# openai/whisper

Hardware: AMD Instinct MI355X
Metric: audio-seconds transcribed per wall-second (large-v3 greedy) (higher is better)
Workload: dtype f16

## Files before the change

### include/whisper_hip.h

```cpp
#ifndef WHISPER_HIP_H
#define WHISPER_HIP_H

#include <stddef.h>
#include <stdint.h>

#ifdef __cplusplus
extern "C" {
#endif

#define WH_ABI_VERSION 1
#define WH_MEL_SCRATCH_BYTES 2048

enum {
  WH_OK = 0,
  WH_ERR_ARG = 1,
  WH_ERR_WORKSPACE = 2,
  WH_ERR_HIP = 3,
  WH_ERR_STATE = 4,
  WH_ERR_LIMIT = 5,
  WH_ERR_HANDOFF = 6,
  WH_RUNNING = 7,
  WH_ERR_STREAM = 8
};

// ... 61 lines not shown
                          int64_t *n_frames_out, int32_t *stats, void *scratch, size_t scratch_bytes, void *stream);

int wh_model_create(const wh_dims *dims, int dtype, const wh_model_weights *weights, wh_model **out);
void wh_model_destroy(wh_model *m);

size_t wh_encoder_workspace_bytes(const wh_model *m, int batch);
int wh_encode(const wh_model *m, const void *mel, int mel_is_f16, int batch, void *out,
              void *workspace, size_t workspace_bytes, void *stream);

enum {
  WH_TASK_CAPTURE_Q = 1,
  WH_TASK_TWO_LAUNCH_SELF = 2,
  WH_TASK_TWO_LAUNCH_CROSS = 4,
  WH_TASK_EXPIRE_HANDOFFS = 16,
  WH_TASK_FUSED_SELF = 32,
  WH_TASK_LN_PROLOGUE = 64
};
size_t wh_task_workspace_bytes(const wh_model *m, int n_audio, int n_group, int max_prefill_tokens,
                               int flags);
int wh_task_create(const wh_model *m, int n_audio, int n_group, int max_prefill_tokens, int flags,
                   void *workspace, size_t workspace_bytes, wh_task **out);
void wh_task_destroy(wh_task *t);
int wh_task_set_audio(wh_task *t, const void *features, void *stream);
int wh_task_prefill(wh_task *t, const int64_t *tokens, int64_t token_stride, int T0,
                    const int32_t *sel_pos, int n_sel, float *logits_out, void *stream);
size_t wh_score_scratch_bytes(const wh_model *m, int n_rows, int n_pos);
int wh_task_score(wh_task *t, const int64_t *tokens, int64_t token_stride, int T0, const int32_t *n_tok,
                  int first, int v_end, float *logprob_out, float *top_logprob_out, int32_t *top_token_out,
                  void *scratch, size_t scratch_bytes, void *stream);
int wh_task_step(wh_task *t, const int64_t *last_tokens, int64_t token_stride, float *logits_out,
                 void *stream);
// ... 89 lines not shown
```

### whisper_amd/csrc/api.cpp

```cpp
#include "../../include/whisper_hip.h"
#include "kernels.h"
#include "flac_core.h"

#include <hip/hip_runtime.h>
#include <math.h>
#include <cmath>
#include <stdlib.h>
#include <string.h>
#include <atomic>
#include <mutex>
#include <new>
#include <vector>

using namespace whk;

static thread_local hipError_t g_last_hip = hipSuccess;

#define HIPCHK(expr)                                   \
  do {                                                 \
    hipError_t _e = (expr);                            \
    if (_e != hipSuccess) { g_last_hip = _e; return WH_ERR_HIP; } \
  } while (0)

extern "C" int wh_abi_version(void) { return WH_ABI_VERSION; }
// ... 207 lines not shown
    HIPCHK(gemm(m, w.att, D, L.out_w, D, w.x, D, M, D, L.out_b, 0, w.x, D, true, s));
    HIPCHK(launch_layernorm(w.x, D, L.mlp_ln_w, L.mlp_ln_b, w.xn, D, M, D, m->dtype, s));
    HIPCHK(gemm(m, w.xn, D, L.fc1_w, D, w.h, 4 * D, M, 4 * D, L.fc1_b, 1, nullptr, 0, false, s));
    HIPCHK(gemm(m, w.h, 4 * D, L.fc2_w, 4 * D, w.x, D, M, D, L.fc2_b, 0, w.x, D, true, s));
  }
  HIPCHK(launch_layernorm(w.x, D, m->w.enc_ln_post_w, m->w.enc_ln_post_b, out, D, M, D, m->dtype, s));
  return WH_OK;
}

struct wh_loop;
struct wh_task {
  const wh_model* m;
  int B, G, R, Tmax, flags;
  int pos;
  bool audio_set;
  int steps_eager[2];
  int handoff_fallbacks;
  hipGraph_t graph[2]; hipGraphExec_t graph_exec[2];
  void* cross_kv;
  void* cross_vt;
  int vt_ld;
  void* self_k; void* self_v;
  void* spare_k; void* spare_v;
  float* x; void* xn; void* qkv; void* att; void* h; void* qbuf;
  void* part_o; float* part_ml;
  float* logits;
  float* xsel; void* xseln;
  int* d_pos; int* d_alive; int* d_sel; int* d_src;
  int* d_lag;
  int* h_lag;
  int* h_poll;
  hipEvent_t poll_event;
  hipEvent_t done_event;
// ... 29 lines not shown
};

enum { LOOP_IDLE = 0, LOOP_GREEDY = 1, LOOP_BEAM = 2 };
enum { PH_STEPPING = 0, PH_DRAINING = 1 };
struct wh_loop {
  int phase;
  hipStream_t s;
  wh_beam_params bp;
  int64_t* tokens; int64_t token_stride; int sot_index, no_speech_token;
  float* sum_logprobs; float* no_speech_probs;
  int64_t* fin_tokens; int32_t* fin_len; float* fin_scores; int32_t* fin_count;
  SampleArgs sa; BeamArgs ba;
  PhraseArgs ph; bool biased;
  RepArgs rep; bool rep_on;
  bool fused_embed, pending, wait_due;
  int ntok, steps, ntok_at_copy, cur;
  int n_tokens;
};

struct TaskGuard {
  wh_task* t; bool ok;
  explicit TaskGuard(wh_task* task, bool loop_call = false) : t(task), ok(false) {
    if (t) {
      int expected = 0; ok = t->busy.compare_exchange_strong(expected, 1);
      if (ok && !loop_call && t->loop_kind != 0) { t->busy.store(0); ok = false; }
    }
  }
  ~TaskGuard() { if (t && ok) t->busy.store(0); }
};
#define TASK_ENTER(task) TaskGuard _guard(task); if ((task) && !_guard.ok) return WH_ERR_STATE
// ... 42 lines not shown
  t->qbuf = c.take(R * D * es);
  size_t Rp = Mx < (size_t)SKINNY_ROWS ? Mx : (size_t)SKINNY_ROWS;
  if (Rp < R) Rp = R;
  if (Rp < 48) Rp = 48;
  t->part_o = c.take(Rp * H * DEC_ATTN_MAX_SPLITS * 64 * 4);
  t->part_ml = (float*)c.take(Rp * H * DEC_ATTN_MAX_SPLITS * 2 * 4);
  t->logits = (float*)c.take(R * 2 * V * 4);
  t->xsel = (float*)c.take(Mx * D * 4);
  t->xseln = c.take(Mx * D * es);
  t->d_pos = (int*)c.take(256);
  t->d_alive = (int*)c.take(256);
  t->d_sel = (int*)c.take(Mx * 4);
  t->d_src = (int*)c.take(R * 4);
  t->d_lag = (int*)c.take(R * 4);
  t->step_tokens = (int64_t*)c.take(R * 8);
  t->samp_part = (float*)c.take(greedy_sample_scratch_bytes((int)R, (int)V));
  t->samp_state = (int*)c.take(R * 16);
  t->phrase_root = (int*)c.take(V * 4);
  t->phrase_span = (int*)c.take(R * 8);
  t->beam_scratch = t->G > 1 ? c.take(beam_scratch_bytes((int)R, (int)V)) : nullptr;
  t->beam_flags = t->G > 1 ? (int*)c.take((2 * (size_t)t->B + 1) * 4) : nullptr;
  t->beam_lcp = t->G > 1 ? (int*)c.take(((size_t)t->B * 64 + R) * 4) : nullptr;
  t->qcap = (t->flags & WH_TASK_CAPTURE_Q) ? c.take(L * R * C * D * es) : nullptr;
  t->xq_gran = (unsigned long long*)c.take(R * (D / 2) * 8);
  t->sq_gran = (unsigned long long*)c.take(R * (3 * D / 2) * 8);
  t->so_gran = (unsigned long long*)c.take(R * (D / 2) * 8);
  t->x2 = (float*)c.take(R * D * 4);
  t->d_tick = (int*)c.take(256);
  t->d_err = t->d_tick + 16;
  t->merge_cnt = (int*)c.take(R * H * 4);
  t->xh = c.take((R + 7) / 8 * 8 * D * 2);
// ... 38 lines not shown
#ifdef WH_DEV
    t->fused_out = t->fused_sattn && (WH_DEV_FLAG("WH_FUSED_OUT") || (flags & 8 ));
#else
    t->fused_out = false;
#endif
  }
  t->h_lag = (int*)calloc((size_t)t->R, sizeof(int));
  if (!t->h_lag) { delete t; return WH_ERR_ARG; }
  t->needs_reset = true;
  t->busy.store(0);
  *out = t;
  return WH_OK;
}

static void drop_step_graphs(wh_task* t) {
  for (int i = 0; i < 2; ++i) {
    if (t->graph_exec[i]) { (void)hipGraphExecDestroy(t->graph_exec[i]); t->graph_exec[i] = nullptr; }
    if (t->graph[i]) { (void)hipGraphDestroy(t->graph[i]); t->graph[i] = nullptr; }
    t->steps_eager[i] = 0;
  }
}

extern "C" void wh_task_destroy(wh_task* t) {
  if (!t) return;
  drop_step_graphs(t);
  free(t->h_lag);
  if (t->h_poll) (void)hipHostFree(t->h_poll);
  if (t->h_sel) (void)hipHostFree(t->h_sel);
  if (t->poll_event) (void)hipEventDestroy(t->poll_event);
  if (t->done_event) (void)hipEventDestroy(t->done_event);
  if (t->sel_event) (void)hipEventDestroy(t->sel_event);
  delete t->loop;
  delete t;
}

extern "C" int wh_task_position(const wh_task* t) { return t ? t->pos : -1; }

extern "C" int wh_task_info(wh_task* t, int what, void* stream) {
  if (!t) return -1;
  if (what == 0) return t->fused_xattn ? 1 : 0;
  if (what == 2) return t->fused_sattn ? 1 : 0;
  if (what == 3) return (t->fused_out || t->fused_xout) ? 1 : 0;
  if (what == 4) return t->handoff_fallbacks;
  if (what == 5) return t->ln_post_sites;
  if (what == 1) {
    if (t->needs_reset) return 0;
    int v = 0;
    if (hipMemcpyAsync(&v, t->d_err, 4, hipMemcpyDeviceToHost, (hipStream_t)stream) != hipSuccess) return -1;
    if (hipStreamSynchronize((hipStream_t)stream) != hipSuccess) return -1;
    return v;
  }
  return -1;
}

static int task_reset_impl(wh_task* t, void* stream_) {
  if (!t) return WH_ERR_ARG;
  hipStream_t s = (hipStream_t)stream_;
  HIPCHK(hipMemsetAsync(t->d_pos, 0, 4, s));
  t->pos = 0;
// ... 430 lines not shown
static SAttnArgs sattn_args(const wh_task* t, int l, int epoch, const float* x_in, float* x_out) {
  const wh_model* m = t->m;
  const wh_dims& d = m->d;
  const int D = d.n_text_state;
  const wh_layer_weights& L = m->dec[l];
  SAttnArgs a; memset(&a, 0, sizeof(a));
  a.xf = x_in; a.xf_ld = D; a.W = L.qkv_w; a.bias = L.qkv_b; a.D = D; a.H = d.n_text_head; a.R = t->R;
  a.out_w = L.out_w; a.out_b = L.out_b; a.x_out = x_out; a.og = t->so_gran;
  a.kcache = self_k_layer(t, l); a.vcache = self_v_layer(t, l); a.cache_bs = (int64_t)d.n_text_ctx * D;
  a.d_pos = t->d_pos; a.lag = t->d_lag; a.q_out = t->qbuf;
  a.out = t->att; a.o_ld = D;
  a.qg = t->sq_gran; a.d_tick = t->d_tick; a.epoch = epoch; a.layer = l; a.err = t->d_err; a.mode = fused_mode(1) | ((t->flags & WH_TASK_EXPIRE_HANDOFFS) ? 4 : 0);
  return a;
}

static int step_launch(wh_task* t, hipStream_t s, bool embedded = false) {
  const wh_model* m = t->m;
  const wh_dims& d = m->d;
  const int D = d.n_text_state, C = d.n_text_ctx, V = d.n_vocab;
  const int R = t->R;
  if (!embedded)
    HIPCHK(launch_embed(t->step_tokens, 1, R, 1, m->w.tok_emb, m->w.dec_pos, t->d_pos, t->d_lag, D, V, t->x, m->dtype, s));
  float* xc = t->x;
  float* xo = t->x2;
  const StepPlan plan = step_plan(t);
  t->ln_post_sites = (int)plan.post_cq + (int)plan.post_fc1;
  for (int l = 0; l < d.n_text_layer; ++l) {
    const wh_layer_weights& L = m->dec[l];
    bool out_done = false;
    if (t->fused_sattn) {
      HIPCHK(launch_sattn8(sattn_args(t, l, 0, xc, t->fused_out ? xo : nullptr), s));
// ... 9 lines not shown
    if (t->fused_xout) out_done = true;
    if (!out_done)
      HIPCHK(gemv_resid(m, plain_proj(t, t->att, D, plan.frag_self, t->self_splits, R, L.out_w, L.out_b, D, D), xc, s,
                        plan.post_cq ? t : nullptr));
    if (t->fused_xattn) {
      HIPCHK(launch_xattn8(xattn_args(t, l, 0, xc, t->fused_xout), s));
    } else {
      HIPCHK(gemv_store(m, ln_site(t, plan.post_cq, false, xc, L.cross_ln_w, L.cross_ln_b, L.cq_w, L.cq_b, D), EPI_STORE, t->qbuf, D, false, s));
      HIPCHK(launch_attn_decode(cross_attn_args(t, l, t->qbuf, R, t->G, t->cross_splits, &plan), m->dtype, s));
    }
    const int rc = launch_cross_out(t, plan, L, xc, s);
    if (rc != WH_OK) return rc;
    HIPCHK(gemv_store(m, ln_site(t, plan.post_fc1, false, xc, L.mlp_ln_w, L.mlp_ln_b, L.fc1_w, L.fc1_b, 4 * D), EPI_GELU, t->h, 4 * D, plan.frag_mlp, s));
    HIPCHK(gemv_resid(m, plain_proj(t, t->h, 4 * D, plan.frag_mlp, 1, R, L.fc2_w, L.fc2_b, D, 4 * D), xc, s));
  }
  GemvArgs g = logits_proj(m, xc, R, t->logits, V);
  g.bump = t->d_pos; g.bump_by = 1;
  g.bump2 = t->d_tick;
  HIPCHK(launch_gemv(g, m->dtype, s));
  return WH_OK;
}

static bool graphs_enabled() {
  static int v = -1;
  if (v < 0) { const char* e = getenv("WH_NO_GRAPH"); v = (e && e[0] == '1') ? 0 : 1; }
  return v == 1;
}

static int step_run(wh_task* t, hipStream_t s, bool embedded = false) {
  if (t->pos <= 0) return WH_ERR_STATE;
  if (t->pos + 1 > t->m->d.n_text_ctx) return WH_ERR_ARG;
  int rc;
  const int gi = embedded ? 1 : 0;
  if (t->graph_exec[gi]) {
    HIPCHK(hipGraphLaunch(t->graph_exec[gi], s));
  } else if (s == nullptr || !graphs_enabled() || t->steps_eager[gi] < 1) {
    rc = step_launch(t, s, embedded);
    if (rc != WH_OK) return rc;
    t->steps_eager[gi]++;
  } else {
    HIPCHK(hipStreamBeginCapture(s, hipStreamCaptureModeThreadLocal));
    rc = step_launch(t, s, embedded);
    hipError_t e = hipStreamEndCapture(s, &t->graph[gi]);
    if (rc != WH_OK) return rc;
    HIPCHK(e);
    HIPCHK(hipGraphInstantiate(&t->graph_exec[gi], t->graph[gi], nullptr, nullptr, 0));
    HIPCHK(hipGraphLaunch(t->graph_exec[gi], s));
  }
  t->pos += 1;
  return WH_OK;
}

extern "C" int wh_task_step(wh_task* t, const int64_t* last_tokens, int64_t token_stride, float* logits_out,
                            void* stream_) {
  TASK_ENTER(t);
  if (!t || !last_tokens || !logits_out) return WH_ERR_ARG;
  hipStream_t s = (hipStream_t)stream_;
// ... 100 lines not shown
  HIPCHK(hipMemcpyAsync(t->h_poll + t->B + HP_ERR0, t->d_err, 4, hipMemcpyDeviceToHost, s));

  int32_t sel[2]; int n_sel;
  const bool want_ns = L->no_speech_token >= 0 && L->no_speech_probs != nullptr;
  if (want_ns && L->sot_index != T0 - 1) { sel[0] = L->sot_index; sel[1] = T0 - 1; n_sel = 2; }
  else { sel[0] = T0 - 1; n_sel = 1; }
  int rc = prefill_impl(t, L->tokens, L->token_stride, T0, sel, n_sel, t->logits, V, s, leaders);
  if (rc != WH_OK) return rc;
  if (leaders) { rc = replicate_leader_rows(t, T0, t->logits, n_sel, s); if (rc != WH_OK) return rc; }
  if (want_ns) HIPCHK(launch_no_speech(t->logits, (int64_t)n_sel * V, R, V, L->no_speech_token, L->no_speech_probs, s));
  HIPCHK(hipMemsetAsync(L->sum_logprobs, 0, (size_t)R * 4, s));
  *n_sel_out = n_sel;
  return WH_OK;
}

static int greedy_start(wh_task* t) {
  wh_loop* L = t->loop;
  hipStream_t s = L->s;
  const wh_greedy_params* p = &L->bp.rules;
  const wh_dims& d = t->m->d;
  const int V = d.n_vocab, R = t->R, T0 = p->sample_begin;
  int* hp = t->h_poll + t->B;
  int n_sel;
  int rc = loop_prompt_pass(t, false, &n_sel);
  if (rc != WH_OK) return rc;
  hp[HP_ALIVE_INIT] = T0 - 1;
  HIPCHK(hipMemcpyAsync(t->d_alive, hp + HP_ALIVE_INIT, 4, hipMemcpyHostToDevice, s));

  SampleArgs& sa = L->sa; memset(&sa, 0, sizeof(sa));
  set_sampling_rules(sa.rules, t, L);
// ... 10 lines not shown
    HIPCHK(hipMemsetAsync(t->phrase_span, 0, (size_t)R * 8, s));
  }
  L->rep_on = t->rep_on; L->rep = t->rep;
  L->fused_embed = !WH_DEV_FLAG("WH_NO_FUSED_EMBED");
  if (L->fused_embed) {
    sa.x_next = t->x; sa.tok_emb = t->m->w.tok_emb; sa.pos_emb = t->m->w.dec_pos; sa.D = d.n_text_state;
    sa.emb_f16 = t->m->dtype == WH_F16 ? 1 : 0; sa.n_pos = d.n_text_ctx;
  }
  if (p->temperature > 0.f) {
    sa.inv_temperature = 1.0f / p->temperature;
    sa.seed_lo = (uint32_t)(p->seed & 0xffffffffu); sa.seed_hi = (uint32_t)(p->seed >> 32);
  }
  sa.rules.logits = t->logits + (size_t)(n_sel - 1) * V; sa.rules.logits_ld = (int64_t)n_sel * V;
  HIPCHK(launch_greedy_sample(sa, s, L->biased ? &ph : nullptr, L->rep_on ? &L->rep : nullptr));
  sa.rules.logits = t->logits; sa.rules.logits_ld = V;
  L->ntok = T0 + 1; L->steps = 1;
  L->pending = L->wait_due = false; L->ntok_at_copy = 0;
  L->phase = PH_STEPPING;
  return WH_OK;
}

static int beam_update(wh_task* t, const float* logits, int64_t logits_ld, int first) {
  wh_loop* L = t->loop;
  const wh_dims& d = t->m->d;
  const size_t es = t->m->esize;
  const int R = t->R, B = t->B, G = t->G;
  const int64_t row_bytes = (int64_t)d.n_text_ctx * d.n_text_state * es;
  int64_t* buf[2] = {L->tokens, L->tokens + (int64_t)R * L->token_stride};
  int* done[2] = {t->beam_flags, t->beam_flags + B};
  BeamArgs& a = L->ba;
// ... 54 lines not shown
      bool finished = false;
      for (;;) {
        if (L->pending && L->wait_due) {
          const int rc = event_reached(t->poll_event, block);
          if (rc != WH_OK) return rc;
          L->pending = L->wait_due = false;
          if (t->loop_kind == LOOP_GREEDY) {
            if (t->h_poll[0] < L->ntok_at_copy - 1) { finished = true; break; }
          } else {
            bool fin = true;
            for (int b = 0; b < B; ++b) fin = fin && t->h_poll[b] != 0;
            if (fin) { finished = true; break; }
          }
        }
        if (!(L->steps < p->max_steps && L->ntok <= p->n_ctx && L->ntok <= d.n_text_ctx)) break;
        int rc = step_run(t, s, t->loop_kind == LOOP_GREEDY && L->fused_embed);
        if (rc != WH_OK) return rc;
        if (t->loop_kind == LOOP_GREEDY) HIPCHK(launch_greedy_sample(L->sa, s, L->biased ? &L->ph : nullptr, L->rep_on ? &L->rep : nullptr));
        else { rc = beam_update(t, t->logits, d.n_vocab, 0); if (rc != WH_OK) return rc; }
        ++L->ntok; ++L->steps;
        if (L->pending && (L->steps & 7) == 2) L->wait_due = true;
        if ((L->steps & 7) == 0) {
          if (t->loop_kind == LOOP_GREEDY) HIPCHK(hipMemcpyAsync(t->h_poll, t->d_alive, 4, hipMemcpyDeviceToHost, s));
          else HIPCHK(hipMemcpyAsync(t->h_poll, (L->cur ? t->beam_flags + B : t->beam_flags), (size_t)B * 4, hipMemcpyDeviceToHost, s));
          HIPCHK(hipEventRecord(t->poll_event, s));
          L->pending = true; L->wait_due = false; L->ntok_at_copy = L->ntok;
        }
      }
      (void)finished;
      if (t->loop_kind == LOOP_GREEDY) {
        HIPCHK(hipMemcpyAsync(hp + HP_ALIVE, t->d_alive, 4, hipMemcpyDeviceToHost, s));
      } else {
        HIPCHK(hipMemcpyAsync(hp + HP_APPLIED, t->beam_flags + 2 * B, 4, hipMemcpyDeviceToHost, s));
// ... 529 lines not shown
```

### whisper_amd/csrc/gemv.hip

```cpp
#include "common.h"
#include "kernels.h"
#include <stdlib.h>

#ifndef WH_GEMV8_MAX_ROWS
#define WH_GEMV8_MAX_ROWS 24
#endif

namespace {

#define ISSUE_FENCE() asm volatile("" ::: "memory")

constexpr int CS = 4;

__device__ __forceinline__ float4v load_part4(const float* p) { return *(const float4v*)p; }
__device__ __forceinline__ float4v load_part4(const half_t* p) {
  const half4v h = *(const half4v*)p;
  return float4v{(float)h[0], (float)h[1], (float)h[2], (float)h[3]};
}

template <typename T> struct Pack4;
template <> struct Pack4<float> {
  static __device__ __forceinline__ void store(float* p, float a, float b, float c, float d) {
    *(float4v*)p = float4v{a, b, c, d};
  }
// ... 1191 lines not shown
bool rows48_applies(const whk::GemvArgs& a) {
  return !WH_DEV_FLAG("WH_NO_ROWS48") && a.R > WH_GEMV8_MAX_ROWS && a.R <= 48 && a.pro == whk::PRO_LN && a.ln_folded &&
         a.K % 256 == 0 && a.K <= 1280 && a.N >= 2048 && a.variant <= 0 &&
         (a.epi == whk::EPI_STORE || a.epi == whk::EPI_GELU || a.epi == whk::EPI_QKV);
}

hipError_t launch_rows48(const whk::GemvArgs& a, hipStream_t stream) {
  whk::g_form = "rows48";
  const size_t lds = (size_t)48 * a.K * 2 > 49152 ? (size_t)48 * a.K * 2 : 49152;
  static whk::LdsAttr attr2;
  { hipError_t e = whk::raise_dynamic_lds(attr2, (const void*)gemv_rows48_kernel<2>, 160 * 1024); if (e != hipSuccess) return e; }
  hipLaunchKernelGGL((gemv_rows48_kernel<2>), dim3((a.N + 31) / 32), dim3(1024), lds, stream, a);
  return hipGetLastError();
}

__global__ __launch_bounds__(1024) void gemv_rows48_stream_kernel(whk::GemvArgs a) {
  extern __shared__ __attribute__((aligned(16))) char smem[];
  pin_kernargs(a);
  constexpr int WAVES = 16, J = 5, NB = 20;
  const int K = a.K, nks = K / 32;
  half_t* xs = (half_t*)smem;
  float* gb = (float*)(smem + (size_t)48 * K * 2);
  const int tid = threadIdx.x, lane = tid & 63;
  const int wave = __builtin_amdgcn_readfirstlane(tid >> 6);
  const int i16 = lane & 15, g4 = lane >> 4;
  const int R = a.R;
  const int ntiles = (a.N + 15) / 16;

  float4v v[3][J];
#pragma unroll
  for (int i = 0; i < 3; ++i) {
    const int r = wave + WAVES * i;
    const float* src = a.xf + (int64_t)(r < R ? r : 0) * a.xf_ld;
#pragma unroll
    for (int j = 0; j < J; ++j) {
      int k = (j * 64 + lane) * 4; if (k > K - 4) k = K - 4;
      v[i][j] = *(const float4v*)(src + k);
    }
  }
  for (int k = tid * 4; k < K; k += 4096) {
    *(float4v*)(gb + k) = *(const float4v*)(a.ln_w + k);
    *(float4v*)(gb + K + k) = *(const float4v*)(a.ln_b + k);
  }
  __syncthreads();
  {
    const float invK = 1.0f / (float)K;
#pragma unroll
    for (int i = 0; i < 3; ++i) {
      const int r = wave + WAVES * i;
      float sum = 0.f;
#pragma unroll
      for (int j = 0; j < J; ++j) {
        const float t = (v[i][j][0] + v[i][j][1]) + (v[i][j][2] + v[i][j][3]);
        sum += ((j * 64 + lane) * 4 < K) ? t : 0.f;
      }
      const float mean = wave_sum(sum) * invK;
      float ss = 0.f;
// ... 11 lines not shown
        const int k = (j * 64 + lane) * 4;
        if (k < K) {
          const float4v w4 = *(const float4v*)(gb + k), b4 = *(const float4v*)(gb + K + k);
          half_t* dst = xr + ((((k >> 3) ^ (r & 15)) << 3) | (k & 7));
          if (r < R)
            Pack4<half_t>::store(dst, (v[i][j][0] - mean) * rstd * w4[0] + b4[0], (v[i][j][1] - mean) * rstd * w4[1] + b4[1],
                                 (v[i][j][2] - mean) * rstd * w4[2] + b4[2], (v[i][j][3] - mean) * rstd * w4[3] + b4[3]);
          else
            Pack4<half_t>::store(dst, 0.f, 0.f, 0.f, 0.f);
        }
      }
    }
  }
  __syncthreads();

  for (int tile = blockIdx.x * WAVES + wave; tile < ntiles; tile += gridDim.x * WAVES) {
    int n = tile * 16 + i16; if (n > a.N - 1) n = a.N - 1;
    const half_t* base = (const half_t*)a.W + (int64_t)n * K + g4 * 8;
    float4v acc[3];
#pragma unroll
    for (int rt = 0; rt < 3; ++rt) acc[rt] = float4v{0.f, 0.f, 0.f, 0.f};
    for (int st0 = 0; st0 < nks; st0 += NB) {
      half8v w[NB];
#pragma unroll
      for (int u = 0; u < NB; ++u) {
        int st = st0 + u; if (st > nks - 1) st = nks - 1;
        w[u] = __builtin_nontemporal_load((const half8v*)(base + st * 32));
      }
#pragma unroll
      for (int u = 0; u < NB; ++u) {
        const int st = st0 + u;
        if (st < nks) {
#pragma unroll
          for (int rt = 0; rt < 3; ++rt) {
            const half8v xf = *(const half8v*)(xs + (size_t)(rt * 16 + i16) * K + (((st * 4 + g4) ^ i16) << 3));
            acc[rt] = __builtin_amdgcn_mfma_f32_16x16x32_f16(w[u], xf, acc[rt], 0, 0, 0);
          }
        }
      }
    }
#pragma unroll
    for (int rt = 0; rt < 3; ++rt) {
      const int row = rt * 16 + i16;
      if (row < R) {
        float* y = (float*)a.y + (int64_t)row * a.y_ld + tile * 16 + g4 * 4;
#pragma unroll
        for (int e = 0; e < 4; ++e)
          if (tile * 16 + g4 * 4 + e < a.N) y[e] = acc[rt][e];
      }
    }
  }
  if (a.bump && blockIdx.x == 0 && tid == 0) atomicAdd(a.bump, a.bump_by);
  if (a.bump2 && blockIdx.x == 0 && tid == 0) atomicAdd(a.bump2, 1);
}

bool rows48_stream_applies(const whk::GemvArgs& a) {
  return !WH_DEV_FLAG("WH_NO_ROWS48") && a.R > 16 && a.R <= 48 && a.pro == whk::PRO_LN && a.epi == whk::EPI_F32 && !a.bias &&
         a.K % 256 == 0 && a.K <= 1280 && a.N >= 16384 && a.variant <= 0;
}

hipError_t launch_rows48_stream(const whk::GemvArgs& a, hipStream_t stream) {
  whk::g_form = "rows48_stream";
  const size_t lds = (size_t)48 * a.K * 2 + (size_t)2 * a.K * 4;
  static whk::LdsAttr attr;
  { hipError_t e = whk::raise_dynamic_lds(attr, (const void*)gemv_rows48_stream_kernel, 160 * 1024); if (e != hipSuccess) return e; }
  const int ntiles = (a.N + 15) / 16;
  int wgs = (ntiles + 15) / 16;
  if (wgs > 256) wgs = 256;
  hipLaunchKernelGGL(gemv_rows48_stream_kernel, dim3(wgs), dim3(1024), lds, stream, a);
  return hipGetLastError();
}

template <typename T, int MS>
__global__ __launch_bounds__(256) void merge_partials_kernel(const T* __restrict__ part_o, const float* __restrict__ part_ml,
                                                             int S, int R, int H, T* __restrict__ out, int64_t o_ld, int o_frag) {
  const int i = blockIdx.x * 256 + threadIdx.x;
  if (i >= R * H * 16) return;
  const int r = i / (H * 16), rem = i - r * (H * 16);
  const int h = rem >> 4, d4 = rem & 15;
  const int64_t pb = (int64_t)r * H + h, ps = (int64_t)R * H;
  float2v ml[MS];
  float4v o[MS];
#pragma unroll
  for (int s = 0; s < MS; ++s) {
// ... 87 lines not shown
  g_form = dtype == 1 ? (splits <= 4 ? "merge<half,4>" : "merge<half,16>") : (splits <= 4 ? "merge<float,4>" : "merge<float,16>");
  if (dtype == 1) {
    if (splits <= 4)
      hipLaunchKernelGGL((merge_partials_kernel<half_t, 4>), grid, block, 0, stream, (const half_t*)part_o, part_ml, splits, R, H, (half_t*)out, o_ld, o_frag);
    else
      hipLaunchKernelGGL((merge_partials_kernel<half_t, DEC_ATTN_MAX_SPLITS>), grid, block, 0, stream, (const half_t*)part_o, part_ml, splits, R, H, (half_t*)out, o_ld, o_frag);
  } else {
    if (splits <= 4)
      hipLaunchKernelGGL((merge_partials_kernel<float, 4>), grid, block, 0, stream, (const float*)part_o, part_ml, splits, R, H, (float*)out, o_ld, o_frag);
    else
      hipLaunchKernelGGL((merge_partials_kernel<float, DEC_ATTN_MAX_SPLITS>), grid, block, 0, stream, (const float*)part_o, part_ml, splits, R, H, (float*)out, o_ld, o_frag);
  }
  return hipGetLastError();
}

}
```

### whisper_amd/csrc/kernels.h

```cpp
#pragma once
#include <hip/hip_runtime.h>
#include <stdint.h>

#ifdef WH_PROBE
#define WH_PROBE_FIELD long long* probe;
#define WH_PROBE_KVHS_FIELD int64_t kv_hs;
#define WH_PROBE_AT(args, wg, i) \
  do { if ((args).probe && threadIdx.x == 0) (args).probe[(size_t)(wg) * 8 + (i)] = clock64(); } while (0)
#else
#define WH_PROBE_FIELD
#define WH_PROBE_KVHS_FIELD
#define WH_PROBE_AT(args, wg, i) do {} while (0)
#endif

#ifdef WH_DEV
#include <stdlib.h>
#define WH_DEV_FLAG(name) ([] { static const bool v = [] { const char* e = getenv(name); return e && e[0] == '1'; }(); return v; }())
#define WH_DEV_INT(name) ([] { static const int v = [] { const char* e = getenv(name); return e ? atoi(e) : 0; }(); return v; }())
#else
#define WH_DEV_FLAG(name) false
#define WH_DEV_INT(name) 0
#endif

#include <atomic>
// ... 193 lines not shown
struct PhraseArgs {
  const int* child_begin;
  const int* child_token;
  const int* child_node;
  const int* root_child;
  int* span;
  int n_nodes, n_edges;
  float boost;
};
constexpr int REP_MAX_NGRAM = 16;
struct RepArgs {
  int ngram;
  float penalty;
};
size_t greedy_sample_scratch_bytes(int R, int V);
hipError_t launch_greedy_sample(const SampleArgs& a, hipStream_t stream, const PhraseArgs* ph = nullptr,
                                const RepArgs* rep = nullptr);
hipError_t launch_phrase_root_table(const int* child_begin, const int* child_token, const int* child_node, int n_edges,
                                    int V, int* root, hipStream_t stream);
hipError_t launch_phrase_span(const int* row_state, const int* child_begin, int n_nodes, int R, int* span, hipStream_t stream);
hipError_t launch_no_speech(const float* logits_row0, int64_t row_stride, int R, int V, int no_speech,
                            float* out, hipStream_t stream);
hipError_t launch_gather_tokens(const int64_t* src, int64_t stride, int R, int64_t* dst, hipStream_t stream);

constexpr int BEAM_KMAX = 9;
struct BeamArgs {
  RuleArgs rules;
  int G, K;
  const int64_t* tokens_in; int64_t* tokens_out;
  float* part_stat; float* part_val; int* part_idx;
// ... 76 lines not shown
```

### whisper_amd/csrc/ktest.cpp

```cpp
#include <string.h>

#include "kernels.h"
#include "logit_rules.h"
#include "sample_noise.h"

using namespace whk;

extern "C" {

const char* wht_last_form() { return g_form; }
void wht_clear_form() { g_form = ""; }
int wht_attn_decode_capacity(int dtype) { return attn_decode_capacity(dtype); }
int wht_gemv8_will_run(int R, int N, int K, int pro) { return gemv8_will_run(R, N, K, pro) ? 1 : 0; }
const char* wht_gemv_family(int dtype, int pro, int epi, int R, int N, int K, int64_t ld, int ln_folded, int has_bias, int splits,
                            int H, int x_frag, int y_frag) {
  static const float some_bias = 0.f;
  GemvArgs a;
  memset(&a, 0, sizeof a);
  a.pro = pro; a.epi = epi; a.R = R; a.N = N; a.K = K; a.x_ld = a.xf_ld = ld; a.ln_folded = ln_folded;
  a.bias = has_bias ? &some_bias : nullptr; a.splits = splits; a.H = H; a.x_frag = x_frag; a.y_frag = y_frag;
  return gemv_family(a, dtype);
}

int wht_gemv(int dtype, int pro, const void* x, int64_t x_ld, const float* xf, int64_t xf_ld, const float* ln_w,
// ... 145 lines not shown
  if (e != hipSuccess) return e;
  return launch_greedy_sample(a, (hipStream_t)stream, &ph, &rep);
}
int wht_greedy_sample(const float* logits, int64_t logits_ld, int R, int V, int64_t* tokens, int64_t token_stride,
                      const int* d_ntok, const int* lag, int sample_begin, int eot, int timestamp_begin, int no_timestamps,
                      int max_initial_ts, int suppress_blank, int blank_token, const uint8_t* suppress_mask,
                      float* sum_logprobs, int64_t* step_tokens, int* d_alive_step, float* partials, size_t partials_bytes,
                      float temperature, uint64_t seed, int* row_state, int n_nodes, int n_edges, const int* child_begin,
                      const int* child_token, const int* child_node, const int* root_child, int* span, float boost,
                      void* stream) {
  return wht_greedy_sample_rep(logits, logits_ld, R, V, tokens, token_stride, d_ntok, lag, sample_begin, eot, timestamp_begin,
                               no_timestamps, max_initial_ts, suppress_blank, blank_token, suppress_mask, sum_logprobs,
                               step_tokens, d_alive_step, partials, partials_bytes, temperature, seed, row_state, n_nodes,
                               n_edges, child_begin, child_token, child_node, root_child, span, boost, 0, 1.0f, stream);
}
void wht_rule_mask(const int64_t* row, int ntok, int lag, int V, int sample_begin, int eot, int timestamp_begin,
                   int no_timestamps, int max_initial_ts, int suppress_blank, int blank_token, const uint8_t* suppress_mask,
                   const int* row_state, uint8_t* mask, int* window) {
  const RuleArgs r = rule_args(nullptr, 0, 1, V, 0, nullptr, nullptr, sample_begin, eot, timestamp_begin, no_timestamps,
                               max_initial_ts, suppress_blank, blank_token, suppress_mask, nullptr);
  const RowPos pos = row_pos_of(r, ntok, lag);
  int last = -1;
  for (int t = 0; t < pos.L && timestamp_begin >= 0; ++t)
    if (row[pos.sample_begin + t] >= timestamp_begin) last = t;
  const TsWindow w = row_state ? ts_window_of_state(r, pos, row_state[0], row_state[1], row_state[2])
                               : ts_window_of_history(r, pos, row, last);
  window[0] = w.last_ts; window[1] = w.pen_ts; window[2] = w.lo; window[3] = w.hi;
  for (int v = 0; v < V; ++v) mask[v] = rule_masked(r, pos, w, v) ? 1 : 0;
}
size_t wht_greedy_sample_scratch_bytes(int R, int V) { return greedy_sample_scratch_bytes(R, V); }
// ... 175 lines not shown
```

### whisper_amd/csrc/sampling.hip

```cpp
#include <string.h>

#include "common.h"
#include "kernels.h"
#include "logit_rules.h"
#include "sample_noise.h"

namespace {

using namespace whk;

constexpr int SCHUNK = 1024;

struct Pick {
  float key = WH_NEG_INF, x = WH_NEG_INF; int idx = 0x7fffffff;
};
__device__ __forceinline__ void pick_merge(Pick& a, float key, float x, int idx) {
  if (idx == 0x7fffffff) return;
  if (a.idx == 0x7fffffff || key > a.key || (key == a.key && idx < a.idx)) { a.key = key; a.x = x; a.idx = idx; }
}
__device__ __forceinline__ void pick_wave_reduce(Pick& a) {
#pragma unroll
  for (int o = 32; o > 0; o >>= 1) {
    const float key = __shfl_xor(a.key, o, 64);
    const float x = __shfl_xor(a.x, o, 64);
// ... 9 lines not shown
    for (int g = 0; g < 2; ++g) {
      pick_wave_reduce(pk[g]);
      if (lane == 0) { key[g][wave] = pk[g].key; x[g][wave] = pk[g].x; idx[g][wave] = pk[g].idx; }
    }
  }
  __device__ __forceinline__ Pick range(int g) const {
    Pick p;
    for (int w = 0; w < 4; ++w) pick_merge(p, key[g][w], x[g][w], idx[g][w]);
    return p;
  }
};
__device__ __forceinline__ float gumbel(uint32_t seed_lo, uint32_t seed_hi, int step, int row, int v) {
  const float u = sample_uniform_of_hash(sample_hash(seed_lo, seed_hi, step, row, v));
  return -logf(-logf(u));
}
constexpr int PSTRIDE = 8;

constexpr int HTILE = 256;
constexpr int HLEAD = 16;
static_assert(whk::REP_MAX_NGRAM - 1 <= HLEAD, "a context must fit in front of a tile");
template <bool SAMPLE, bool BIAS, bool REP>
__global__ __launch_bounds__(256) void greedy_partial_kernel(whk::SampleArgs a, int nchunk, whk::PhraseArgs ph, whk::RepArgs rp) {
  pin_kernargs(a);
  if constexpr (BIAS) pin_kernargs(ph);
  if constexpr (REP) pin_kernargs(rp);
  asm volatile("" ::"s"(nchunk));
  __shared__ int sh_hist[REP ? HLEAD + HTILE : 1];
  __shared__ int sh_suffix[REP ? HLEAD : 1];
  __shared__ unsigned sh_pen[REP ? SCHUNK / 32 : 1], sh_ban[REP ? SCHUNK / 32 : 1];
  __shared__ BlockStats<!SAMPLE> sh_st;
  __shared__ BlockPicks sh_pk;
// ... 311 lines not shown
  if (ph) {
    if (!ph->child_begin || !ph->child_token || !ph->child_node || !ph->root_child || !ph->span || !a.row_state ||
        ph->n_nodes < 1 || ph->n_edges < 0)
      return hipErrorInvalidValue;
    if (sample) greedy_sample_launch<true, true>(a, *ph, rep, nchunk, stream);
    else greedy_sample_launch<false, true>(a, *ph, rep, nchunk, stream);
  } else {
    PhraseArgs none;
    memset(&none, 0, sizeof(none));
    if (sample) greedy_sample_launch<true, false>(a, none, rep, nchunk, stream);
    else greedy_sample_launch<false, false>(a, none, rep, nchunk, stream);
  }
  return hipGetLastError();
}

hipError_t launch_phrase_root_table(const int* child_begin, const int* child_token, const int* child_node, int n_edges,
                                    int V, int* root, hipStream_t stream) {
  if (!child_begin || !child_token || !child_node || !root || n_edges < 1 || V < 1) return hipErrorInvalidValue;
  hipError_t e = hipMemsetAsync(root, 0xff, (size_t)V * 4, stream);
  if (e != hipSuccess) return e;
  hipLaunchKernelGGL(phrase_root_table_kernel, dim3((n_edges + 255) / 256), dim3(256), 0, stream, child_begin, child_token,
                     child_node, n_edges, V, root);
  return hipGetLastError();
}

hipError_t launch_phrase_span(const int* row_state, const int* child_begin, int n_nodes, int R, int* span, hipStream_t stream) {
  if (!row_state || !child_begin || !span || n_nodes < 1 || R < 1) return hipErrorInvalidValue;
  hipLaunchKernelGGL(phrase_span_kernel, dim3((R + 63) / 64), dim3(64), 0, stream, row_state, child_begin, n_nodes, R, span);
  return hipGetLastError();
}
// ... 14 lines not shown
```

### whisper_amd/hip.py

```python
from __future__ import annotations

import contextlib
import ctypes as C
import os
import threading
from typing import Dict, List, NamedTuple, Optional, Sequence, Tuple

import torch

_LIB = None
_LIB_PATH = os.environ.get("WHISPER_AMD_LIB") or os.path.join(os.path.dirname(os.path.abspath(__file__)), "libwhisper_hip.so")

WH_F32, WH_F16 = 0, 1
WH_TASK_CAPTURE_Q = 1
WH_TASK_TWO_LAUNCH_SELF = 2
WH_TASK_TWO_LAUNCH_CROSS = 4
WH_TASK_EXPIRE_HANDOFFS = 16
WH_TASK_FUSED_SELF = 32
WH_TASK_LN_PROLOGUE = 64
WH_WEIGHTS_DEC_LN_FOLDED = 1
WH_WEIGHTS_ENC_QK_SCALED = 2
ENC_QK_SCALE = (0.125 * 1.4426950408889634) ** 0.5
MEL_SCRATCH_BYTES = 2048
WH_PCM_U8, WH_PCM_S16, WH_PCM_S32, WH_PCM_F32, WH_PCM_F64 = 0, 1, 2, 3, 4
RESAMPLE_MAX_TAPS = 1 << 23


class HipError(RuntimeError):
    pass


class HipLimitError(HipError):
    """status 5 (WH_ERR_LIMIT): the arguments are valid but exceed a compiled-in limit of the library"""

# ... 682 lines not shown
    def fused_cross_attention(self) -> bool:
        return lib().wh_task_info(self.handle, 0, None) == 1

    @property
    def fused_self_attention(self) -> bool:
        return lib().wh_task_info(self.handle, 2, None) == 1

    @property
    def handoff_fallbacks(self) -> int:
        return lib().wh_task_info(self.handle, 4, None)

    @property
    def ln_post_sites(self) -> int:
        return lib().wh_task_info(self.handle, 5, None)

    def handoff_timeouts(self) -> int:
        with self._call():
            n = lib().wh_task_info(self.handle, 1, stream_ptr(self.stream))
        return n

    def greedy(self, tokens: torch.Tensor, params: GreedyParams, sot_index: int, no_speech_token: int):
        assert tokens.is_cuda and tokens.dtype == torch.int64 and tokens.stride(1) == 1
        dev = tokens.device
        sum_lp = torch.empty(self.n_rows, dtype=torch.float32, device=dev)
        nsp = torch.empty(self.n_rows, dtype=torch.float32, device=dev) if no_speech_token >= 0 else None
        n_out = C.c_int32(0)
        with self._call():
            check(lib().wh_task_greedy(self.handle, C.byref(params), tokens.data_ptr(), tokens.stride(0), sot_index,
                                       no_speech_token, sum_lp.data_ptr(), _ptr(nsp), C.byref(n_out),
                                       stream_ptr(self.stream)), "wh_task_greedy")
# ... 395 lines not shown
```

Baseline: 1181.

## Fuse greedy logit-rule masking and max/logsumexp stats into logits GEMV epilogue

In greedy f16 decoding with 17-48 rows, the logits projection kernel can now apply the suppression and timestamp rules and compute per-chunk max, argmax and sum-exp partials in its epilogue, without writing the full logits matrix. A small final kernel then merges the per-chunk partials to pick tokens. The step graph gets a third variant without the logits GEMV, which is launched eagerly with stats, and the old path stays behind a flag. This removes the full-vocabulary logits write and re-read plus a separate sampling pass. In exchange the GEMV needs extra LDS and per-element rule evaluation, and some work now runs outside the captured graph.

```diff
diff --git a/include/whisper_hip.h b/include/whisper_hip.h
--- a/include/whisper_hip.h
+++ b/include/whisper_hip.h
@@ -99,7 +99,8 @@
   WH_TASK_TWO_LAUNCH_CROSS = 4,
   WH_TASK_EXPIRE_HANDOFFS = 16,
   WH_TASK_FUSED_SELF = 32,
-  WH_TASK_LN_PROLOGUE = 64
+  WH_TASK_LN_PROLOGUE = 64,
+  WH_TASK_THREE_LAUNCH_TAIL = 128
 };
 size_t wh_task_workspace_bytes(const wh_model *m, int n_audio, int n_group, int max_prefill_tokens,
                                int flags);
diff --git a/whisper_amd/csrc/api.cpp b/whisper_amd/csrc/api.cpp
--- a/whisper_amd/csrc/api.cpp
+++ b/whisper_amd/csrc/api.cpp
@@ -245,9 +245,11 @@
   int B, G, R, Tmax, flags;
   int pos;
   bool audio_set;
-  int steps_eager[2];
+  int steps_eager[3];
   int handoff_fallbacks;
-  hipGraph_t graph[2]; hipGraphExec_t graph_exec[2];
+  int tail_fused_steps;
+  const float* x_last;
+  hipGraph_t graph[3]; hipGraphExec_t graph_exec[3];
   void* cross_kv;
   void* cross_vt;
   int vt_ld;
@@ -307,6 +309,7 @@
   PhraseArgs ph; bool biased;
   RepArgs rep; bool rep_on;
   bool fused_embed, pending, wait_due;
+  int tail_chunks;
   int ntok, steps, ntok_at_copy, cur;
   int n_tokens;
 };
@@ -379,7 +382,7 @@
   t->d_src = (int*)c.take(R * 4);
   t->d_lag = (int*)c.take(R * 4);
   t->step_tokens = (int64_t*)c.take(R * 8);
-  t->samp_part = (float*)c.take(greedy_sample_scratch_bytes((int)R, (int)V));
+  t->samp_part = (float*)c.take(std::max(greedy_sample_scratch_bytes((int)R, (int)V), R > 16 && R <= 48 ? logits_stats_scratch_bytes((int)R) : 0));
   t->samp_state = (int*)c.take(R * 16);
   t->phrase_root = (int*)c.take(V * 4);
   t->phrase_span = (int*)c.take(R * 8);
@@ -448,7 +451,7 @@
 }
 
 static void drop_step_graphs(wh_task* t) {
-  for (int i = 0; i < 2; ++i) {
+  for (int i = 0; i < 3; ++i) {
     if (t->graph_exec[i]) { (void)hipGraphExecDestroy(t->graph_exec[i]); t->graph_exec[i] = nullptr; }
     if (t->graph[i]) { (void)hipGraphDestroy(t->graph[i]); t->graph[i] = nullptr; }
     t->steps_eager[i] = 0;
@@ -477,6 +480,7 @@
   if (what == 3) return (t->fused_out || t->fused_xout) ? 1 : 0;
   if (what == 4) return t->handoff_fallbacks;
   if (what == 5) return t->ln_post_sites;
+  if (what == 6) return t->tail_fused_steps;
   if (what == 1) {
     if (t->needs_reset) return 0;
     int v = 0;
@@ -937,7 +941,14 @@
   return a;
 }
 
-static int step_launch(wh_task* t, hipStream_t s, bool embedded = false) {
+static GemvArgs step_logits_proj(const wh_task* t, const float* x) {
+  GemvArgs g = logits_proj(t->m, x, t->R, t->logits, t->m->d.n_vocab);
+  g.bump = t->d_pos; g.bump_by = 1;
+  g.bump2 = t->d_tick;
+  return g;
+}
+
+static int step_launch(wh_task* t, hipStream_t s, bool embedded = false, bool tail = true) {
   const wh_model* m = t->m;
   const wh_dims& d = m->d;
   const int D = d.n_text_state, C = d.n_text_ctx, V = d.n_vocab;
@@ -977,10 +988,8 @@
     HIPCHK(gemv_store(m, ln_site(t, plan.post_fc1, false, xc, L.mlp_ln_w, L.mlp_ln_b, L.fc1_w, L.fc1_b, 4 * D), EPI_GELU, t->h, 4 * D, plan.frag_mlp, s));
     HIPCHK(gemv_resid(m, plain_proj(t, t->h, 4 * D, plan.frag_mlp, 1, R, L.fc2_w, L.fc2_b, D, 4 * D), xc, s));
   }
-  GemvArgs g = logits_proj(m, xc, R, t->logits, V);
-  g.bump = t->d_pos; g.bump_by = 1;
-  g.bump2 = t->d_tick;
-  HIPCHK(launch_gemv(g, m->dtype, s));
+  t->x_last = xc;
+  if (tail) HIPCHK(launch_gemv(step_logits_proj(t, xc), m->dtype, s));
   return WH_OK;
 }
 
@@ -990,20 +999,21 @@
   return v == 1;
 }
 
-static int step_run(wh_task* t, hipStream_t s, bool embedded = false) {
+static int step_run(wh_task* t, hipStream_t s, bool embedded = false, bool tail = true) {
   if (t->pos <= 0) return WH_ERR_STATE;
   if (t->pos + 1 > t->m->d.n_text_ctx) return WH_ERR_ARG;
+  if (!tail && !embedded) return WH_ERR_ARG;
   int rc;
-  const int gi = embedded ? 1 : 0;
+  const int gi = !tail ? 2 : embedded ? 1 : 0;
   if (t->graph_exec[gi]) {
     HIPCHK(hipGraphLaunch(t->graph_exec[gi], s));
   } else if (s == nullptr || !graphs_enabled() || t->steps_eager[gi] < 1) {
-    rc = step_launch(t, s, embedded);
+    rc = step_launch(t, s, embedded, tail);
     if (rc != WH_OK) return rc;
     t->steps_eager[gi]++;
   } else {
     HIPCHK(hipStreamBeginCapture(s, hipStreamCaptureModeThreadLocal));
-    rc = step_launch(t, s, embedded);
+    rc = step_launch(t, s, embedded, tail);
     hipError_t e = hipStreamEndCapture(s, &t->graph[gi]);
     if (rc != WH_OK) return rc;
     HIPCHK(e);
@@ -1134,6 +1144,22 @@
   return WH_OK;
 }
 
+static int tail_select(const wh_task* t, const wh_loop* L) {
+  if ((t->flags & WH_TASK_THREE_LAUNCH_TAIL) || t->m->dtype != WH_F16 || !L->fused_embed) return 0;
+  if (L->bp.rules.temperature > 0.f || L->biased || L->rep_on) return 0;
+  return logits_stats_chunks(step_logits_proj(t, t->x), t->m->dtype);
+}
+static int greedy_tail_fused(wh_task* t, hipStream_t s) {
+  const wh_loop* L = t->loop;
+  LogitStatArgs sx; memset(&sx, 0, sizeof(sx));
+  sx.rules = L->sa.rules; sx.row_state = L->sa.row_state; sx.partials = L->sa.partials;
+  sx.ntok = t->pos;
+  HIPCHK(launch_logits_stats(step_logits_proj(t, t->x_last), sx, t->m->dtype, s));
+  HIPCHK(launch_greedy_final(L->sa, L->tail_chunks, s));
+  t->tail_fused_steps++;
+  return WH_OK;
+}
+
 static int greedy_start(wh_task* t) {
   wh_loop* L = t->loop;
   hipStream_t s = L->s;
@@ -1174,6 +1200,7 @@
   sa.rules.logits = t->logits + (size_t)(n_sel - 1) * V; sa.rules.logits_ld = (int64_t)n_sel * V;
   HIPCHK(launch_greedy_sample(sa, s, L->biased ? &ph : nullptr, L->rep_on ? &L->rep : nullptr));
   sa.rules.logits = t->logits; sa.rules.logits_ld = V;
+  L->tail_chunks = tail_select(t, L);
   L->ntok = T0 + 1; L->steps = 1;
   L->pending = L->wait_due = false; L->ntok_at_copy = 0;
   L->phase = PH_STEPPING;
@@ -1258,9 +1285,11 @@
           }
         }
         if (!(L->steps < p->max_steps && L->ntok <= p->n_ctx && L->ntok <= d.n_text_ctx)) break;
-        int rc = step_run(t, s, t->loop_kind == LOOP_GREEDY && L->fused_embed);
+        const bool tail_fused = t->loop_kind == LOOP_GREEDY && L->tail_chunks > 0;
+        int rc = step_run(t, s, t->loop_kind == LOOP_GREEDY && L->fused_embed, !tail_fused);
         if (rc != WH_OK) return rc;
-        if (t->loop_kind == LOOP_GREEDY) HIPCHK(launch_greedy_sample(L->sa, s, L->biased ? &L->ph : nullptr, L->rep_on ? &L->rep : nullptr));
+        if (tail_fused) { rc = greedy_tail_fused(t, s); if (rc != WH_OK) return rc; }
+        else if (t->loop_kind == LOOP_GREEDY) HIPCHK(launch_greedy_sample(L->sa, s, L->biased ? &L->ph : nullptr, L->rep_on ? &L->rep : nullptr));
         else { rc = beam_update(t, t->logits, d.n_vocab, 0); if (rc != WH_OK) return rc; }
         ++L->ntok; ++L->steps;
         if (L->pending && (L->steps & 7) == 2) L->wait_due = true;
diff --git a/whisper_amd/csrc/gemv.hip b/whisper_amd/csrc/gemv.hip
--- a/whisper_amd/csrc/gemv.hip
+++ b/whisper_amd/csrc/gemv.hip
@@ -1,5 +1,6 @@
 #include "common.h"
 #include "kernels.h"
+#include "logit_rules.h"
 #include <stdlib.h>
 
 #ifndef WH_GEMV8_MAX_ROWS
@@ -1229,7 +1230,10 @@
   return hipGetLastError();
 }
 
-__global__ __launch_bounds__(1024) void gemv_rows48_stream_kernel(whk::GemvArgs a) {
+constexpr int RS48_RULE_BYTES = 48 * 32;
+constexpr int RS48_STAT_BYTES = 16 * 48 * 2 * 12;
+template <bool STATS>
+__device__ __forceinline__ void rows48_stream_body(const whk::GemvArgs& a, const whk::LogitStatArgs* sx) {
   extern __shared__ __attribute__((aligned(16))) char smem[];
   pin_kernargs(a);
   constexpr int WAVES = 16, J = 5, NB = 20;
@@ -1241,6 +1245,21 @@
   const int i16 = lane & 15, g4 = lane >> 4;
   const int R = a.R;
   const int ntiles = (a.N + 15) / 16;
+  whk::RowPos* sh_pos = (whk::RowPos*)(smem + (size_t)48 * K * 2 + (size_t)2 * K * 4);
+  whk::TsWindow* sh_win = (whk::TsWindow*)(sh_pos + 48);
+  float* sh_stat = (float*)((char*)sh_pos + RS48_RULE_BYTES);
+  int rs_lag = 0, rs0 = 0, rs1 = 0, rs2 = 0;
+  if constexpr (STATS) {
+    pin_kernargs(*sx);
+    if (tid < 48) {
+      const int rr = tid < R ? tid : 0;
+      if (sx->rules.lag) rs_lag = load_agent_int(sx->rules.lag + rr);
+      if (sx->rules.timestamp_begin >= 0) {
+        rs0 = load_agent_int(sx->row_state + 4 * rr); rs1 = load_agent_int(sx->row_state + 4 * rr + 1);
+        rs2 = load_agent_int(sx->row_state + 4 * rr + 2);
+      }
+    }
+  }
 
   float4v v[3][J];
 #pragma unroll
@@ -1256,6 +1275,13 @@
   for (int k = tid * 4; k < K; k += 4096) {
     *(float4v*)(gb + k) = *(const float4v*)(a.ln_w + k);
     *(float4v*)(gb + K + k) = *(const float4v*)(a.ln_b + k);
+  }
+  if constexpr (STATS) {
+    if (tid < 48) {
+      const whk::RowPos p = whk::row_pos_of(sx->rules, sx->ntok, rs_lag);
+      sh_pos[tid] = p;
+      sh_win[tid] = whk::ts_window_of_state(sx->rules, p, rs0, rs1, rs2);
+    }
   }
   __syncthreads();
   {
@@ -1297,9 +1323,28 @@
   }
   __syncthreads();
 
+  if constexpr (STATS) {
+    if (g4 == 0) {
+#pragma unroll
+      for (int q = 0; q < 6; ++q) {
+        float* o = sh_stat + ((wave * 48 + (q >> 1) * 16 + i16) * 2 + (q & 1)) * 3;
+        o[0] = WH_NEG_INF; o[1] = 0.f; o[2] = __int_as_float(whk::NO_IDX);
+      }
+    }
+  }
   for (int tile = blockIdx.x * WAVES + wave; tile < ntiles; tile += gridDim.x * WAVES) {
     int n = tile * 16 + i16; if (n > a.N - 1) n = a.N - 1;
     const half_t* base = (const half_t*)a.W + (int64_t)n * K + g4 * 8;
+    uint8_t sup[4] = {0, 0, 0, 0};
+    if constexpr (STATS) {
+      if (sx->rules.suppress_mask) {
+#pragma unroll
+        for (int e = 0; e < 4; ++e) {
+          int vv = tile * 16 + g4 * 4 + e; if (vv > a.N - 1) vv = a.N - 1;
+          sup[e] = sx->rules.suppress_mask[vv];
+        }
+      }
+    }
     float4v acc[3];
 #pragma unroll
     for (int rt = 0; rt < 3; ++rt) acc[rt] = float4v{0.f, 0.f, 0.f, 0.f};
@@ -1322,24 +1367,107 @@
         }
       }
     }
-#pragma unroll
-    for (int rt = 0; rt < 3; ++rt) {
-      const int row = rt * 16 + i16;
-      if (row < R) {
-        float* y = (float*)a.y + (int64_t)row * a.y_ld + tile * 16 + g4 * 4;
-#pragma unroll
-        for (int e = 0; e < 4; ++e)
-          if (tile * 16 + g4 * 4 + e < a.N) y[e] = acc[rt][e];
-      }
+    if constexpr (STATS) {
+      whk::RuleArgs rn = sx->rules;
+      rn.suppress_mask = nullptr;
+      const int split = rn.timestamp_begin >= 0 ? rn.timestamp_begin : a.N;
+#pragma unroll
+      for (int rt = 0; rt < 3; ++rt) {
+        if (rt * 16 >= R) continue;
+        const int row = rt * 16 + i16, rr = row < R ? row : 0;
+        const whk::RowPos pos = sh_pos[rr];
+        const whk::TsWindow win = sh_win[rr];
+        float m[2] = {WH_NEG_INF, WH_NEG_INF};
+        int id[2] = {whk::NO_IDX, whk::NO_IDX};
+        unsigned live = 0;
+#pragma unroll
+        for (int e = 0; e < 4; ++e) {
+          const int vv = tile * 16 + g4 * 4 + e;
+          const bool masked = row >= R || vv >= a.N || sup[e] != 0 || whk::rule_masked(rn, pos, win, vv);
+          const float xv = acc[rt][e];
+          if (!masked && xv != WH_NEG_INF) {
+            live |= 1u << e;
+            const int g = vv < split ? 0 : 1;
+            if (xv > m[g]) { m[g] = xv; id[g] = vv; }
+          }
+        }
+#pragma unroll
+        for (int g = 0; g < 2; ++g) {
+#pragma unroll
+          for (int o = 16; o <= 32; o <<= 1) {
+            const float mo = __shfl_xor(m[g], o, 64);
+            const int io = __shfl_xor(id[g], o, 64);
+            if (mo > m[g] || (mo == m[g] && io < id[g])) { m[g] = mo; id[g] = io; }
+          }
+        }
+        float s[2] = {0.f, 0.f};
+#pragma unroll
+        for (int e = 0; e < 4; ++e) {
+          if ((live >> e) & 1u) {
+            const int g = tile * 16 + g4 * 4 + e < split ? 0 : 1;
+            s[g] += expf(acc[rt][e] - m[g]);
+          }
+        }
+#pragma unroll
+        for (int g = 0; g < 2; ++g) {
+          s[g] += __shfl_xor(s[g], 16, 64);
+          s[g] += __shfl_xor(s[g], 32, 64);
+          if (g4 == 0 && row < R) {
+            float* o = sh_stat + ((wave * 48 + row) * 2 + g) * 3;
+            whk::Stat<true> run{o[0], o[1], __float_as_int(o[2])};
+            whk::stat_merge(run, whk::Stat<true>{m[g], s[g], id[g]});
+            o[0] = run.m; o[1] = run.s; o[2] = __int_as_float(run.idx);
+          }
+        }
+      }
+    } else {
+#pragma unroll
+      for (int rt = 0; rt < 3; ++rt) {
+        const int row = rt * 16 + i16;
+        if (row < R) {
+          float* y = (float*)a.y + (int64_t)row * a.y_ld + tile * 16 + g4 * 4;
+#pragma unroll
+          for (int e = 0; e < 4; ++e)
+            if (tile * 16 + g4 * 4 + e < a.N) y[e] = acc[rt][e];
+        }
+      }
+    }
+  }
+  if constexpr (STATS) {
+    __syncthreads();
+    if (tid < 96 && (tid >> 1) < R) {
+      whk::Stat<true> t[WAVES];
+#pragma unroll
+      for (int w = 0; w < WAVES; ++w) {
+        const float* o = sh_stat + (w * 96 + tid) * 3;
+        t[w] = whk::Stat<true>{o[0], o[1], __float_as_int(o[2])};
+      }
+#pragma unroll
+      for (int d = 1; d < WAVES; d <<= 1) {
+#pragma unroll
+        for (int w = 0; w < WAVES; w += 2 * d) whk::stat_merge(t[w], t[w + d]);
+      }
+      float* o = sx->partials + (((int64_t)(tid >> 1) * sx->nchunk + blockIdx.x) * 2 + (tid & 1)) * whk::STAT_PSTRIDE;
+      o[0] = t[0].m; o[1] = t[0].s; o[2] = __int_as_float(t[0].idx);
     }
   }
   if (a.bump && blockIdx.x == 0 && tid == 0) atomicAdd(a.bump, a.bump_by);
   if (a.bump2 && blockIdx.x == 0 && tid == 0) atomicAdd(a.bump2, 1);
+}
+__global__ __launch_bounds__(1024) void gemv_rows48_stream_kernel(whk::GemvArgs a) { rows48_stream_body<false>(a, nullptr); }
+__global__ __launch_bounds__(1024) void gemv_rows48_stream_stats_kernel(whk::GemvArgs a, whk::LogitStatArgs sx) {
+  rows48_stream_body<true>(a, &sx);
 }
 
 bool rows48_stream_applies(const whk::GemvArgs& a) {
   return !WH_DEV_FLAG("WH_NO_ROWS48") && a.R > 16 && a.R <= 48 && a.pro == whk::PRO_LN && a.epi == whk::EPI_F32 && !a.bias &&
          a.K % 256 == 0 && a.K <= 1280 && a.N >= 16384 && a.variant <= 0;
+}
+
+int rows48_stream_wgs(int N) {
+  const int ntiles = (N + 15) / 16;
+  const int wgs = (ntiles + 15) / 16;
+  return wgs > 256 ? 256 : wgs;
 }
 
 hipError_t launch_rows48_stream(const whk::GemvArgs& a, hipStream_t stream) {
@@ -1347,10 +1475,7 @@
   const size_t lds = (size_t)48 * a.K * 2 + (size_t)2 * a.K * 4;
   static whk::LdsAttr attr;
   { hipError_t e = whk::raise_dynamic_lds(attr, (const void*)gemv_rows48_stream_kernel, 160 * 1024); if (e != hipSuccess) return e; }
-  const int ntiles = (a.N + 15) / 16;
-  int wgs = (ntiles + 15) / 16;
-  if (wgs > 256) wgs = 256;
-  hipLaunchKernelGGL(gemv_rows48_stream_kernel, dim3(wgs), dim3(1024), lds, stream, a);
+  hipLaunchKernelGGL(gemv_rows48_stream_kernel, dim3(rows48_stream_wgs(a.N)), dim3(1024), lds, stream, a);
   return hipGetLastError();
 }
 
@@ -1468,4 +1593,23 @@
   return hipGetLastError();
 }
 
-}
+int logits_stats_chunks(const GemvArgs& a, int dtype) {
+  return dtype == 1 && pick_family(a, dtype) == Family::rows48_stream ? rows48_stream_wgs(a.N) : 0;
+}
+size_t logits_stats_scratch_bytes(int R) { return (size_t)R * 256 * 2 * STAT_PSTRIDE * sizeof(float); }
+
+hipError_t launch_logits_stats(const GemvArgs& a, const LogitStatArgs& sx_, int dtype, hipStream_t stream) {
+  LogitStatArgs sx = sx_;
+  sx.nchunk = logits_stats_chunks(a, dtype);
+  if (sx.nchunk < 1 || !sx.partials || sx.rules.R != a.R || sx.rules.V != a.N || sx.ntok < 0) return hipErrorInvalidValue;
+  if (sx.rules.timestamp_begin >= 0 && !sx.row_state) return hipErrorInvalidValue;
+  g_form = "rows48_stream/stats";
+  const size_t lds = (size_t)48 * a.K * 2 + (size_t)2 * a.K * 4 + RS48_RULE_BYTES + RS48_STAT_BYTES;
+  if (lds > 160 * 1024) return hipErrorInvalidValue;
+  static LdsAttr attr;
+  { hipError_t e = raise_dynamic_lds(attr, (const void*)gemv_rows48_stream_stats_kernel, 160 * 1024); if (e != hipSuccess) return e; }
+  hipLaunchKernelGGL(gemv_rows48_stream_stats_kernel, dim3(sx.nchunk), dim3(1024), lds, stream, a, sx);
+  return hipGetLastError();
+}
+
+}
diff --git a/whisper_amd/csrc/kernels.h b/whisper_amd/csrc/kernels.h
--- a/whisper_amd/csrc/kernels.h
+++ b/whisper_amd/csrc/kernels.h
@@ -231,6 +231,18 @@
   float penalty;
 };
 size_t greedy_sample_scratch_bytes(int R, int V);
+constexpr int STAT_PSTRIDE = 8;
+struct LogitStatArgs {
+  RuleArgs rules;
+  const int* row_state;
+  float* partials;
+  int ntok;
+  int nchunk;
+};
+int logits_stats_chunks(const GemvArgs& a, int dtype);
+size_t logits_stats_scratch_bytes(int R);
+hipError_t launch_logits_stats(const GemvArgs& a, const LogitStatArgs& sx, int dtype, hipStream_t stream);
+hipError_t launch_greedy_final(const SampleArgs& a, int nchunk, hipStream_t stream);
 hipError_t launch_greedy_sample(const SampleArgs& a, hipStream_t stream, const PhraseArgs* ph = nullptr,
                                 const RepArgs* rep = nullptr);
 hipError_t launch_phrase_root_table(const int* child_begin, const int* child_token, const int* child_node, int n_edges,
diff --git a/whisper_amd/csrc/ktest.cpp b/whisper_amd/csrc/ktest.cpp
--- a/whisper_amd/csrc/ktest.cpp
+++ b/whisper_amd/csrc/ktest.cpp
@@ -183,6 +183,44 @@
                                step_tokens, d_alive_step, partials, partials_bytes, temperature, seed, row_state, n_nodes,
                                n_edges, child_begin, child_token, child_node, root_child, span, boost, 0, 1.0f, stream);
 }
+size_t wht_logits_stats_scratch_bytes(int R) { return logits_stats_scratch_bytes(R); }
+int wht_logits_stats(int store, const float* xf, int64_t xf_ld, const float* ln_w, const float* ln_b, const void* W, int V,
+                     int K, int R, float* logits, int64_t logits_ld, int ntok, const int* lag, int sample_begin, int eot,
+                     int timestamp_begin, int no_timestamps, int max_initial_ts, int suppress_blank, int blank_token,
+                     const uint8_t* suppress_mask, const int* row_state, float* partials, size_t partials_bytes,
+                     int* nchunk_out, void* stream) {
+  GemvArgs a;
+  memset(&a, 0, sizeof a);
+  a.pro = PRO_LN; a.xf = xf; a.xf_ld = xf_ld; a.ln_w = ln_w; a.ln_b = ln_b; a.W = W; a.N = V; a.K = K; a.R = R;
+  a.epi = EPI_F32; a.y = logits; a.y_ld = logits_ld;
+  const int nchunk = logits_stats_chunks(a, 1);
+  if (nchunk < 1) return hipErrorInvalidValue;
+  if (store) return launch_gemv(a, 1, (hipStream_t)stream);
+  if (!nchunk_out || partials_bytes < logits_stats_scratch_bytes(R)) return hipErrorInvalidValue;
+  LogitStatArgs sx;
+  memset(&sx, 0, sizeof sx);
+  sx.rules = rule_args(nullptr, 0, R, V, 0, nullptr, lag, sample_begin, eot, timestamp_begin, no_timestamps, max_initial_ts,
+                       suppress_blank, blank_token, suppress_mask, nullptr);
+  sx.row_state = row_state; sx.partials = partials; sx.ntok = ntok;
+  *nchunk_out = nchunk;
+  return launch_logits_stats(a, sx, 1, (hipStream_t)stream);
+}
+int wht_greedy_decide(int nchunk, const float* logits, int64_t logits_ld, int R, int V, int64_t* tokens, int64_t token_stride,
+                      const int* d_ntok, const int* lag, int sample_begin, int eot, int timestamp_begin, int no_timestamps,
+                      int max_initial_ts, int suppress_blank, int blank_token, const uint8_t* suppress_mask,
+                      float* sum_logprobs, int64_t* step_tokens, int* d_alive_step, float* partials, size_t partials_bytes,
+                      int* row_state, float* x_next, const void* tok_emb, const float* pos_emb, int D, int n_pos, void* stream) {
+  if (R < 1 || V < 1 || nchunk < 0) return hipErrorInvalidValue;
+  if (partials_bytes < (nchunk > 0 ? (size_t)R * nchunk * 2 * STAT_PSTRIDE * sizeof(float) : greedy_sample_scratch_bytes(R, V)))
+    return hipErrorInvalidValue;
+  SampleArgs a;
+  memset(&a, 0, sizeof a);
+  a.rules = rule_args(logits, logits_ld, R, V, token_stride, d_ntok, lag, sample_begin, eot, timestamp_begin, no_timestamps,
+                      max_initial_ts, suppress_blank, blank_token, suppress_mask, sum_logprobs);
+  a.tokens = tokens; a.step_tokens = step_tokens; a.d_alive_step = d_alive_step; a.partials = partials; a.row_state = row_state;
+  a.x_next = x_next; a.tok_emb = tok_emb; a.pos_emb = pos_emb; a.D = D; a.emb_f16 = 1; a.n_pos = n_pos;
+  return nchunk > 0 ? launch_greedy_final(a, nchunk, (hipStream_t)stream) : launch_greedy_sample(a, (hipStream_t)stream);
+}
 void wht_rule_mask(const int64_t* row, int ntok, int lag, int V, int sample_begin, int eot, int timestamp_begin,
                    int no_timestamps, int max_initial_ts, int suppress_blank, int blank_token, const uint8_t* suppress_mask,
                    const int* row_state, uint8_t* mask, int* window) {
diff --git a/whisper_amd/csrc/sampling.hip b/whisper_amd/csrc/sampling.hip
--- a/whisper_amd/csrc/sampling.hip
+++ b/whisper_amd/csrc/sampling.hip
@@ -47,7 +47,7 @@
   const float u = sample_uniform_of_hash(sample_hash(seed_lo, seed_hi, step, row, v));
   return -logf(-logf(u));
 }
-constexpr int PSTRIDE = 8;
+constexpr int PSTRIDE = whk::STAT_PSTRIDE;
 
 constexpr int HTILE = 256;
 constexpr int HLEAD = 16;
@@ -389,6 +389,15 @@
   return hipGetLastError();
 }
 
+hipError_t launch_greedy_final(const SampleArgs& a, int nchunk, hipStream_t stream) {
+  if (!a.partials || nchunk < 1 || a.inv_temperature > 0.f) return hipErrorInvalidValue;
+  if (a.rules.timestamp_begin >= 0 && !a.row_state) return hipErrorInvalidValue;
+  PhraseArgs none;
+  memset(&none, 0, sizeof(none));
+  hipLaunchKernelGGL(HIP_KERNEL_NAME(greedy_final_kernel<false, false>), dim3(a.rules.R), dim3(256), 0, stream, a, nchunk, none);
+  return hipGetLastError();
+}
+
 hipError_t launch_phrase_root_table(const int* child_begin, const int* child_token, const int* child_node, int n_edges,
                                     int V, int* root, hipStream_t stream) {
   if (!child_begin || !child_token || !child_node || !root || n_edges < 1 || V < 1) return hipErrorInvalidValue;
diff --git a/whisper_amd/hip.py b/whisper_amd/hip.py
--- a/whisper_amd/hip.py
+++ b/whisper_amd/hip.py
@@ -18,6 +18,7 @@
 WH_TASK_EXPIRE_HANDOFFS = 16
 WH_TASK_FUSED_SELF = 32
 WH_TASK_LN_PROLOGUE = 64
+WH_TASK_THREE_LAUNCH_TAIL = 128
 WH_WEIGHTS_DEC_LN_FOLDED = 1
 WH_WEIGHTS_ENC_QK_SCALED = 2
 ENC_QK_SCALE = (0.125 * 1.4426950408889634) ** 0.5
@@ -730,6 +731,10 @@
     def ln_post_sites(self) -> int:
         return lib().wh_task_info(self.handle, 5, None)
 
+    @property
+    def tail_fused_steps(self) -> int:
+        return lib().wh_task_info(self.handle, 6, None)
+
     def handoff_timeouts(self) -> int:
         with self._call():
             n = lib().wh_task_info(self.handle, 1, stream_ptr(self.stream))
```

Result: no change. 1182, median of 6 (+0.1%).
